# martinruenz/co-fusion

Measured on AMD Instinct MI355X. Metric: frames/sec at 640x480 (N active models) + ICP-reduce achieved HBM GB/s vs peak, higher is better.
Workload: dtype f32

## Files before the change

### co_fusion_amd/api.py

```python
from __future__ import annotations

import ctypes as C

import numpy as np
import torch

from . import lib as _libmod

NUM_PYRS = 3


class Cam(C.Structure):
    _fields_ = [("fx", C.c_float), ("fy", C.c_float), ("cx", C.c_float), ("cy", C.c_float)]

    def level(self, l):
        d = float(1 << l)
        return Cam(self.fx / d, self.fy / d, self.cx / d, self.cy / d)


class Config(C.Structure):
    _fields_ = [("width", C.c_int), ("height", C.c_int), ("fx", C.c_float), ("fy", C.c_float), ("cx", C.c_float),
                ("cy", C.c_float), ("device", C.c_int), ("max_models", C.c_int), ("max_surfels", C.c_int)]


# ... 231 lines not shown
                                         _f(np.asarray(kinv).reshape(9)), _f(np.asarray(krlr).reshape(9)), cols, rows,
                                         A, b, res, sums))
        return (np.array(A, np.float32).reshape(3, 3), np.array(b, np.float32), np.array(res, np.float32),
                np.array(sums, np.int64))

    def gn_solve_step(self, systems, next_level, last_of_level, icp_fix=32):
        arr = systems if isinstance(systems, C.Array) else (GnSystem * len(systems))(*systems)
        self._check(self.lib.cf_gn_solve_step(self.h, len(arr), arr, int(next_level), int(bool(last_of_level)), int(icp_fix)))
        return arr

    def set_icp_launch(self, threads, ppt):
        self._check(self.lib.cf_set_icp_launch(self.h, threads, ppt))

    def set_gn_mode(self, mode):
        self._check(self.lib.cf_set_gn_mode(self.h, int(mode)))

    def track_batch(self, odoms, poses, rgb_only=False, icp_weight=10.0, pyramid=True, fast_odom=False, so3=True, err_surfaces=None):
        n = len(odoms)
        keep = [_f(np.asarray(p, np.float32).reshape(16)) for p in poses]
        pp = (C.POINTER(C.c_float) * max(n, 1))(*[C.cast(k, C.POINTER(C.c_float)) for k in keep])
        oo = (C.c_void_p * max(n, 1))(*[o.h for o in odoms])
        ee = None
        if err_surfaces is not None:
            ee = (C.c_void_p * max(n, 1))(*[e.data_ptr() if e is not None else None for e in err_surfaces])
        opts = TrackOpts(int(rgb_only), int(pyramid), int(fast_odom), int(so3), icp_weight)
        self._check(self.lib.cf_odom_track_batch_async(self.h, oo, n, pp, C.byref(opts), ee))

    def _batch_args(self, odoms, poses):
        n = len(odoms)
        self._keep_poses = [_f(np.asarray(p, np.float32).reshape(16)) for p in poses]
# ... 376 lines not shown
```

### co_fusion_amd/csrc/cabi.hip

```cpp
#include <stdlib.h>
#include <string.h>

#include <string>

#include "cf_host.h"

using namespace cf;

void cf_ctx::set_error(const std::string& m)
{
    std::lock_guard<std::mutex> lk(error_mutex);
    last_error = m;
}

static int lane_ready(cf_ctx* ctx, int lane)
{
    if (!ctx->lanes[lane]) {
        HIPCHK(ctx, hipStreamCreateWithFlags(&ctx->lanes[lane], hipStreamNonBlocking));
        HIPCHK(ctx, hipEventCreateWithFlags(&ctx->lane_done[lane], hipEventDisableTiming));
    }
    return CF_OK;
}
static void leave_lane(cf_ctx* ctx)
{
// ... 23 lines not shown
    ctx->icp_launch = IcpLaunch{256, 0, 0};
    if (int r = dmalloc(ctx, &ctx->d_acc_a, (size_t)kGroups * 32)) return r;
    if (int r = dmalloc(ctx, &ctx->d_acc_b, (size_t)kGroups * 32)) return r;
    if (int r = dmalloc(ctx, &ctx->d_out, 64)) return r;
    if (int r = dmalloc(ctx, &ctx->d_scratch_state, 1)) return r;
    if (int r = dmalloc(ctx, &ctx->d_state_pool, (size_t)cf_ctx::kStateSlots)) return r;
    HIPCHK(ctx, hipHostMalloc(reinterpret_cast<void**>(&ctx->h_state_pool), sizeof(OdomDev) * cf_ctx::kStateSlots, hipHostMallocCoherent));
    memset(ctx->h_state_pool, 0, sizeof(OdomDev) * cf_ctx::kStateSlots);
    if (int r = dmalloc(ctx, &ctx->d_so3_sync, (size_t)ctx->cfg.max_models + 1)) return r;
    if (const char* e = getenv("CF_ICP_ARITH")) {
        if (cf_set_icp_arith(ctx, (!strcmp(e, "gram") || !strcmp(e, "1")) ? CF_ICP_ARITH_GRAM : (!strcmp(e, "reference") || !strcmp(e, "2")) ? CF_ICP_ARITH_REFERENCE
                                  : (!strcmp(e, "product") || !strcmp(e, "0")) ? CF_ICP_ARITH_PRODUCT : -1) != CF_OK) {
            ctx->set_error("CF_ICP_ARITH: product | gram | reference"); return CF_EINVAL;
        }
    }
    if (int r = dmalloc(ctx, &ctx->d_cand_scratch, (size_t)cfg->width * cfg->height)) return r;
    HIPCHK(ctx, hipHostMalloc(reinterpret_cast<void**>(&ctx->h_scratch_state), sizeof(OdomDev)));
    HIPCHK(ctx, hipHostMalloc(reinterpret_cast<void**>(&ctx->h_out), sizeof(unsigned long long) * 64));
    ctx->prof.capacity = 8192;
    ctx->prof.events = new hipEvent_t[ctx->prof.capacity];
    for (int i = 0; i < ctx->prof.capacity; i++) HIPCHK(ctx, hipEventCreate(&ctx->prof.events[i]));
    ctx->prof.used = 0; ctx->prof.enabled = 0; ctx->prof.bytes = 0; ctx->prof.launches = 0;
    HIPCHK(ctx, hipStreamSynchronize(ctx->stream));
    return CF_OK;
}

void cf_destroy(cf_ctx* ctx)
{
    if (ctx && ctx->batch_event) (void)hipEventDestroy(ctx->batch_event);
    if (ctx) for (int i = 0; i < cf_ctx::kSurfEvents; i++) if (ctx->surf_events[i]) (void)hipEventDestroy(ctx->surf_events[i]);
// ... 237 lines not shown
```

### co_fusion_amd/csrc/cabi_track.hip

```cpp
#include <math.h>
#include <stdio.h>
#include <stdlib.h>
#include <string.h>

#include <string>
#include <utility>

#include "cf_host.h"

using namespace cf;

#ifdef CF_ABLATE
static bool diag_no_box() { static const bool v = getenv("CF_NO_SCREEN_BOX") != nullptr; return v; }
static bool diag_no_zcull() { static const bool v = getenv("CF_NO_ZCULL") != nullptr; return v; }
static bool diag_no_occ() { static const bool v = getenv("CF_NO_OCC") != nullptr; return v; }
static const char* diag_icp_ablate() { return getenv("CF_ICP_ABLATE"); }
static const char* diag_trace_out(const char* name) { const char* e = getenv("CF_ICP_TRACE_OUT"); return e ? e : name; }
struct DiagCall {
    const char* name; int call = -2, seen = 0;
    bool hit() { if (call == -2) call = getenv(name) ? atoi(getenv(name)) : -1; return call >= 0 && seen++ == call; }
};
static int clear_accumulators(cf_ctx* ctx, cf_odom* const* ods, int n)
{
    for (int m = 0; m < n; m++) {
// ... 235 lines not shown
    GnHook hook{};
    hook.fn = ctx->collective; hook.user = ctx->collective_user;
    bool any_split = false;
    for (int m = 0; m < n; m++) { hook.split[m] = ods[m]->band_end > 0 ? 1 : 0; any_split = any_split || hook.split[m]; }
    if (any_split && !ctx->collective) { ctx->set_error("a tracker has a row band (cf_odom_set_band) but no collective is registered (cf_set_collective)"); return CF_ESTATE; }
    if (any_split && ctx->gn_mode == 0) { ctx->set_error("split reductions need the record-slot data path (cf_set_gn_mode 1)"); return CF_ESTATE; }
    cf::ProfSink* prof = nullptr;
    if (ctx->prof.enabled > 0 && (ctx->prof_calls++ % (unsigned)ctx->prof.enabled) == 0) prof = &ctx->prof;
    TrackDiag diag;
    if (int r = diag.begin(ctx)) return r;
    LaunchShape* shapes[kMaxBatch];
    for (int m = 0; m < n; m++) shapes[m] = &ods[m]->launch_shape;
    IcpLaunch launch_cfg = ctx->icp_launch; launch_cfg.shape = shapes;
    if (!launch_gn_track(ctx->stream, launch_cfg, states, ctx->d_so3_sync, any_split ? &hook : nullptr, icp_args, rgb_args, n,
                         ctx->cfg.width, ctx->cfg.height, opts->so3 != 0, opts->pyramid != 0, opts->fast_odom != 0, terms.rgb, terms.icp, ctx->gn_mode, prof,
                         h_states, prep_fused ? &prep : nullptr)) {
        ctx->set_error("tracking: the registered collective failed inside the Gauss-Newton loop");
        return CF_ESTATE;
    }
    LAUNCHCHK(ctx);
    if (int r = diag.end(ctx, ods, n, icp_args[0], rgb_args[0])) return r;
    for (int m = 0; m < n; m++) ods[m]->result_pending = true;
    return CF_OK;
}

int cf_wait_stream(cf_ctx* ctx)
{
    HIPCHK(ctx, hipStreamSynchronize(ctx->stream));
    return CF_OK;
}

// ... 43 lines not shown
            for (int r = k + 1; r < N; r++) lu[r * N + k] /= lu[k * N + k];
        for (int r = k + 1; r < N; r++)
            for (int c = k + 1; c < N; c++) lu[r * N + c] -= lu[r * N + k] * lu[k * N + c];
    }
    for (int j = 0; j < N; j++) {
        double x[N];
        for (int i = 0; i < N; i++) x[i] = (perm[i] == j) ? 1.0 : 0.0;
        for (int i = 0; i < N; i++)
            for (int c = 0; c < i; c++) x[i] -= lu[i * N + c] * x[c];
        for (int i = N - 1; i >= 0; i--) {
            for (int c = i + 1; c < N; c++) x[i] -= lu[i * N + c] * x[c];
            x[i] /= lu[i * N + i];
        }
        for (int i = 0; i < N; i++) cov[i * N + j] = x[i];
    }
    return CF_OK;
}

int cf_set_gn_mode(cf_ctx* ctx, int mode)
{
    if (!ctx || mode < 0 || mode > 2) return CF_EINVAL;
    if (mode == 2) {
        if (ctx->xcd_round_robin < 0) { HIPCHK(ctx, hipStreamSynchronize(ctx->stream)); ctx->xcd_round_robin = probe_xcd_round_robin(ctx->stream) ? 1 : 0; }
        if (!ctx->xcd_round_robin) { ctx->set_error("cf_set_gn_mode 2: workgroups of a launch are not dealt round-robin over 8 XCDs on this device; the mode needs that"); return CF_ESTATE; }
    }
    if (mode != ctx->gn_mode) {
        ctx->gn_mode_epoch++;
    }
    ctx->gn_mode = mode;
    return CF_OK;
// ... 38 lines not shown
```

### co_fusion_amd/csrc/cf_host.h

```cpp
#pragma once

#include <string.h>

#include <mutex>
#include <string>

#include "cf_kernels.h"

struct cf_ctx;
struct cf_thread_binding { const cf_ctx* ctx = nullptr; hipStream_t stream = nullptr; };
extern thread_local cf_thread_binding cf_tls_binding;

struct cf_ctx {
    cf_config cfg{};
    hipStream_t stream = nullptr;
    hipStream_t cur() const { return cf_tls_binding.ctx == this ? cf_tls_binding.stream : stream; }
    hipStream_t own_stream = nullptr;
    std::string last_error;
    std::mutex error_mutex;
    cf::IcpLaunch icp_launch{256, 0};
    int icp_arith = 0;
    float* d_ref = nullptr;
    float* h_ref = nullptr;
    unsigned long long* d_acc_a = nullptr;
    unsigned long long* d_acc_b = nullptr;
    unsigned long long* d_out = nullptr;
    unsigned long long* h_out = nullptr;
    cf::OdomDev* d_scratch_state = nullptr;
    cf::OdomDev* h_scratch_state = nullptr;
    uint8_t* d_cand_scratch = nullptr;
    cf::So3Sync* d_so3_sync = nullptr;
    unsigned gn_mode_epoch = 0;
    int xcd_round_robin = -1;
    int gn_mode = 1;
    static constexpr int kStateSlots = 256;
    cf::OdomDev* d_state_pool = nullptr;
    cf::OdomDev* h_state_pool = nullptr;
    bool slot_used[kStateSlots]{};
    hipEvent_t batch_event = nullptr;
    bool extent_cull = true;
    static constexpr int kLanes = 8;
    hipStream_t lanes[kLanes]{};
    hipEvent_t lane_done[kLanes]{};
    hipEvent_t fork_point = nullptr;
    static constexpr int kMarks = 64;
    hipEvent_t marks[kMarks]{};
    bool mark_set[kMarks]{};
    hipStream_t forked_from = nullptr;
    bool forked = false;
    unsigned lanes_used = 0;
    int (*collective)(void* user, int op, void* dev_buf, uint64_t words, void* stream) = nullptr;
    void* collective_user = nullptr;
    void* rccl = nullptr;
    unsigned prof_calls = 0;
// ... 106 lines not shown
```

### co_fusion_amd/csrc/cf_kernels.h

```cpp
#pragma once

#include <hip/hip_runtime.h>
#include <hip/hip_ext.h>
#include <stdint.h>

#include "../../include/cofusion_hip.h"

namespace cf {

__host__ __device__ __forceinline__ cf_cam cam_level(cf_cam c, int level)
{
    const int div = 1 << level;
    return cf_cam{c.fx / div, c.fy / div, c.cx / div, c.cy / div};
}

constexpr int kGroups = 64;

struct alignas(64) GnHot {
    int icp, level_done; float cull_z[2];
    float Rcurr[9], tcurr[3];
    float Rprev_inv[9], tprev[3];
    int cull_box[4];
    int rgb, rgbOnly, level_done2, pad;
    float krkInv[9], kt[3];
// ... 215 lines not shown
void launch_rgb_residual(hipStream_t s, const RgbArgs& ra, int n);
void launch_rgb_step(hipStream_t s, const RgbArgs& ra, int n);
constexpr uint64_t kRgbResidualBytes = 27;
constexpr uint64_t kRgbResidualBytesCompact = 11;
void launch_acc_total(hipStream_t s, const unsigned long long* acc, unsigned long long* out);
void launch_rgb_cand(hipStream_t s, const int16_t* dIdx, const int16_t* dIdy, const float* next_depth,
                     const uint8_t* next_image, float min_scale, int cols, int rows, uint8_t* cand);
void launch_so3_step(hipStream_t s, const uint8_t* last_image, const uint8_t* next_image, const float basis[9],
                     const float kinv[9], const float krlr[9], int cols, int rows, unsigned long long* out16);
void launch_gn_solve(hipStream_t s, const GnArgs& gn, int n, int next_level, int last_of_level);

struct ProfSink {
    hipEvent_t* events; int capacity; int used; uint64_t bytes; uint64_t launches; int enabled;
};

constexpr int kSo3Blocks = 16;
constexpr int kStepSubs = 16;
struct So3Sync { unsigned long long acc[10][16]; unsigned arrive, depart;
                 unsigned step_top, pad;
                 unsigned step_sub[kStepSubs][32]; };
struct GnHook { int (*fn)(void* user, int op, void* dev_buf, uint64_t words, void* stream); void* user; int split[kMaxBatch]; };
struct TrackerStates { OdomDev* dev[kMaxBatch]; const OdomDev* host[kMaxBatch]; };
bool launch_gn_track(hipStream_t s, IcpLaunch cfg, const TrackerStates& states, So3Sync* so3_syncs ,
                     const GnHook* hook, const IcpArgs icp_args[3], const RgbArgs rgb_args[3], int n, int width, int height, bool so3,
                     bool pyramid, bool fast_odom, bool rgb, bool icp, int mode, ProfSink* prof,
                     OdomDev* const* h_states = nullptr ,
                     const RgbPrepBatch* prep = nullptr );
void rgb_prep_levels(RgbPrepBatch& b, int n, int W, int H);
float replay_icp_level0(hipStream_t s, IcpLaunch cfg, const IcpArgs& a0, const RgbArgs& r0, int n, int slots, int ablate, int reps, hipEvent_t e0, hipEvent_t e1);
#ifdef CF_ABLATE
void trace_so3_dump(hipStream_t s);
void trace_solve_begin();
void trace_solve_end(hipStream_t s, const char* path);
void trace_step_solve(hipStream_t s, IcpLaunch cfg, const IcpArgs& a0, const RgbArgs& r0, So3Sync* syncs, int n, const char* path);
void trace_icp_level0(hipStream_t s, IcpLaunch cfg, const IcpArgs& a0, const RgbArgs& r0, int n, int slots, const char* path);
#endif
bool probe_xcd_round_robin(hipStream_t s);
float sqrt_gate_lt(float T);
float sqrt_gate_le(float T);

constexpr int kSurfBatch = 16;
struct IndexPassArgs {
// ... 116 lines not shown
```

### co_fusion_amd/csrc/track_reduce.hip

```cpp
#include "cf_device.h"
#include "cf_kernels.h"
#include "track_prep_dev.h"
#include "track_sums_dev.h"

namespace cf {

__device__ __forceinline__ int idiv(int n, IDiv d) { return (int)(__umulhi((unsigned)n, d.M) >> d.s); }

struct IcpProj { f3 vcurr_g; int g; int inb; int ux, uy; };

__device__ __forceinline__ IcpProj icp_project(const m33& Rcurr, const f3& tcurr, const m33& Rprev_inv, const f3& tprev, const cf_cam& intr,
                                               int cols, int rows, f3 vcurr)
{
    IcpProj o;
    o.vcurr_g = mul(Rcurr, vcurr) + tcurr;
    const f3 vcurr_cp = mul(Rprev_inv, o.vcurr_g - tprev);
    const int ux = f2i_rn(vcurr_cp.x * intr.fx / vcurr_cp.z + intr.cx);
    const int uy = f2i_rn(vcurr_cp.y * intr.fy / vcurr_cp.z + intr.cy);
    o.inb = !(ux < 0 || uy < 0 || ux >= cols || uy >= rows || vcurr_cp.z < 0);
    o.g = o.inb ? uy * cols + ux : 0;
    o.ux = o.inb ? ux : 0; o.uy = o.inb ? uy : 0;
    return o;
}

// ... 660 lines not shown
    g_last_icp_args = args; g_last_n_icp_blocks = n_icp_blocks; g_last_grid = (int)grid.x;
#endif
    const unsigned lds = cfg.gram ? (unsigned)(cfg.threads / 64) * kGramWaveDwords * sizeof(int) : 0u;
    const int tag = (level == 0 ? 0 : level == 1 ? 1 : 2) + (n > 1 ? 4 : 0), ppt_index = cfg.ppt == 4 ? 2 : cfg.ppt == 2 ? 1 : 0;
    static_assert(kIcpKernels[3][0][0] == nullptr && kIcpKernels[2][2][1] && kIcpKernels[4][0][0], "tags are level (0..2) or level + 4: row 3 is never looked up");
    launch_plain_or_timed(kIcpKernels[tag][ppt_index][cfg.gram ? 1 : 0], grid, dim3(cfg.threads), lds, s, ev0, ev1, args, ra, n_icp_blocks);
}

void launch_icp_level(hipStream_t s, IcpLaunch cfg, const IcpArgs& args, int n, int level, hipEvent_t ev0, hipEvent_t ev1)
{
    launch_icp_rgbres(s, cfg, args, RgbArgs{}, true, false, n, level, ev0, ev1);
}

bool launch_gn_track(hipStream_t s, IcpLaunch cfg, const TrackerStates& states, So3Sync* so3_syncs, const GnHook* hook, const IcpArgs icp_args[3],
                     const RgbArgs rgb_args[3], int n, int width, int height, bool so3, bool pyramid, bool fast_odom, bool rgb, bool icp, int mode,
                     ProfSink* prof, OdomDev* const* h_states, const RgbPrepBatch* prep)
{
    int iterations[3];
    iterations[0] = fast_odom ? 3 : 10;
    iterations[1] = pyramid ? 5 : 0;
    iterations[2] = pyramid ? 4 : 0;
    int first_level = 2;
    while (first_level > 0 && iterations[first_level] == 0) first_level--;
    {
        const int gx = so3 ? 8 * kSo3Blocks : 1;
        static const RgbPrepBatch none{};
        const int prep_bx = prep ? prep->m[0].L.blk_end[2] : 0;
        so3_prealign_kernel<<<gx * n + prep_bx * n, 256, 0, s>>>(states, so3_syncs, so3 ? 1 : 0, first_level, gx, gx * n, prep ? *prep : none, prep_bx);
    }
    GnArgs gn{};
    gn.icp_gram = cfg.gram;
    gn.slot_px = cfg.threads * 4;
    for (int m = 0; m < n; m++) {
        gn.od[m] = const_cast<OdomDev*>(icp_args[0].m[m].st);
        gn.icp_acc[m] = icp_args[0].m[m].acc;
        gn.rgb_acc[m] = rgb_args[0].m[m].rgb_acc;
        gn.od_host[m] = h_states ? h_states[m] : nullptr;
    }
    const bool slots = mode != 0;
    bool any_culled = false;
    for (int m = 0; m < n; m++) any_culled = any_culled || (icp_args[0].m[m].cull && icp_args[0].m[m].err);
    const bool err_aside = icp && any_culled;
    bool hook_failed = false;
// ... 211 lines not shown
```

### co_fusion_amd/csrc/track_so3_dev.h

```cpp
#pragma once
#include "track_prep_dev.h"
#include "track_sums_dev.h"

namespace cf {

__device__ __forceinline__ void screen_box(const float* lo, const float* hi, const float* Rb, const float* tb, const float* Rcurr, const float* tcurr,
                                           cf_cam intr, float distThres, int W, int H, int lane, int (&out)[4], float (&zout)[2])
{
    const float finf = __int_as_float(0x7f800000);
    zout[0] = -finf; zout[1] = finf;
    if (!(lo[0] <= hi[0])) { out[0] = 1; out[1] = 1; out[2] = 0; out[3] = 0; return; }
    const float m = distThres * 1.01f + 1e-3f;
    const float px = (lane & 1) ? hi[0] + 3.f : lo[0] - 3.f, py = (lane & 2) ? hi[1] + 3.f : lo[1] - 3.f;
    const float znear = lo[2] - m, pz = (lane & 4) ? hi[2] + m : znear;
    const float cx_ = (px - intr.cx) / intr.fx * pz, cy_ = (py - intr.cy) / intr.fy * pz;
    const float dx = (Rb[0] * cx_ + Rb[1] * cy_ + Rb[2] * pz + tb[0]) - tcurr[0];
    const float dy = (Rb[3] * cx_ + Rb[4] * cy_ + Rb[5] * pz + tb[1]) - tcurr[1];
    const float dz = (Rb[6] * cx_ + Rb[7] * cy_ + Rb[8] * pz + tb[2]) - tcurr[2];
    const float xc = Rcurr[0] * dx + Rcurr[3] * dy + Rcurr[6] * dz;
    const float yc = Rcurr[1] * dx + Rcurr[4] * dy + Rcurr[7] * dz;
    const float zc = Rcurr[2] * dx + Rcurr[5] * dy + Rcurr[8] * dz;
    const float u = intr.fx * xc / zc + intr.cx, v = intr.fy * yc / zc + intr.cy;
    const bool bad = !(znear > 0.05f) || !(zc > 0.05f) || !is_finite(u) || !is_finite(v);
    float u0 = u, u1 = u, v0 = v, v1 = v, z0 = zc, z1 = zc;
// ... 7 lines not shown
    zout[0] = z0 - (1e-3f + 1e-3f * fabsf(z0)); zout[1] = z1 + (1e-3f + 1e-3f * fabsf(z1));
    const float fw = (float)(W + 16), fh = (float)(H + 16);
    out[0] = (int)floorf(fminf(fmaxf(u0, -16.f), fw)) - 3; out[1] = (int)floorf(fminf(fmaxf(v0, -16.f), fh)) - 3;
    out[2] = (int)ceilf(fminf(fmaxf(u1, -16.f), fw)) + 3; out[3] = (int)ceilf(fminf(fmaxf(v1, -16.f), fh)) + 3;
}

__device__ __forceinline__ void so3_gradient(const uint8_t* __restrict__ img, int cols, int x, int y, float& gx, float& gy)
{
    const float actu = (float)img[y * cols + x];
    float back = (float)img[y * cols + x - 1], fore = (float)img[y * cols + x + 1];
    gx = ((back + actu) / 2.0f) - ((fore + actu) / 2.0f);
    back = (float)img[(y - 1) * cols + x]; fore = (float)img[(y + 1) * cols + x];
    gy = ((back + actu) / 2.0f) - ((fore + actu) / 2.0f);
}

__device__ __forceinline__ void so3_pass(const uint8_t* __restrict__ lastImage, const uint8_t* __restrict__ nextImage,
                                         const m33& B, const m33& Ki, const float* __restrict__ krlr, int cols, int rows,
                                         unsigned long long (*lds)[16], unsigned long long* totals, int block, int blocks)
{
    constexpr float lim = (float)(1 << ((50 - kFixSO3) / 2));
    constexpr float scale = (float)(1 << kFixSO3);
    const int N = cols * rows, T = blockDim.x;
    unsigned long long acc[16];
#pragma unroll
    for (int k = 0; k < 16; k++) acc[k] = 0;
    const float a = krlr[0], b = krlr[1], c = krlr[2], d = krlr[3], e = krlr[4], f = krlr[5], g = krlr[6], h = krlr[7],
                ii = krlr[8];
    for (int k = block * T + threadIdx.x; k < N; k += blocks * T) {
        const int y = k / cols, x = k - y * cols;
        const f3 unwarped = {(float)x, (float)y, 1.0f};
        const f3 warped = mul(B, unwarped);
        const int wx = f2i_rn(warped.x / warped.z), wy = f2i_rn(warped.y / warped.z);
        if (!(wx >= 1 && wx < cols - 1 && wy >= 1 && wy < rows - 1 && x >= 1 && x < cols - 1 && y >= 1 && y < rows - 1))
            continue;
        float gnx, gny, glx, gly;
        so3_gradient(nextImage, cols, wx, wy, gnx, gny);
        so3_gradient(lastImage, cols, x, y, glx, gly);
        const float gx = (gnx + glx) / 2.0f, gy = (gny + gly) / 2.0f;
        const f3 point = mul(Ki, unwarped);
        const float z2 = point.z * point.z;
        const f3 left = {((point.z * (d * gy + a * gx)) - (gy * g * y) - (gx * g * x)) / z2,
                         ((point.z * (e * gy + b * gx)) - (gy * h * y) - (gx * h * x)) / z2,
                         ((point.z * (f * gy + c * gx)) - (gy * ii * y) - (gx * ii * x)) / z2};
        const f3 jac = cross(left, point);
        const float row[4] = {jac.x, jac.y, jac.z, -((float)nextImage[wy * cols + wx] - (float)lastImage[y * cols + x])};
        double r[4], rs[4];
#pragma unroll
        for (int q = 0; q < 4; q++) { r[q] = (double)clamp_row(row[q], lim); rs[q] = (double)(clamp_row(row[q], lim) * scale); }
#pragma unroll
        for (int p = 0; p < 3; p++)
#pragma unroll
            for (int q = 0; q < 4; q++)
                if (q >= p)
                    acc[4 * p - (p * (p - 1)) / 2 + (q - p)] += (unsigned long long)__double_as_longlong(fma(rs[p], r[q], kMagic)) - kMagicBits;
        acc[9] += (unsigned long long)__double_as_longlong(fma(rs[3], r[3], kMagic)) - kMagicBits;
        acc[10] += 1;
    }
    const int lane = threadIdx.x & 63, wave = threadIdx.x >> 6;
    const unsigned long long v = wave_reduce16_u64(acc, lane);
    if ((lane & 3) == 0) lds[wave][lane >> 2] = v;
    __syncthreads();
    if (threadIdx.x < 16) {
        unsigned long long t = 0;
        for (int w = 0; w < (T >> 6); w++) t += lds[w][threadIdx.x];
        totals[threadIdx.x] = t;
    }
    __syncthreads();
}

__device__ inline void so3_unpack(const unsigned long long* t, float A[9], float b[3], float residual[2])
{
    int shift = 0;
    for (int i = 0; i < 3; ++i)
        for (int j = i; j < 4; ++j) {
            const float value = fix_to_f32((long long)t[shift++], kFixSO3);
            if (j == 3) b[i] = value;
            else A[j * 3 + i] = A[i * 3 + j] = value;
        }
    residual[0] = fix_to_f32((long long)t[9], kFixSO3);
    residual[1] = (float)(long long)t[10];
}

// ... 22 lines not shown
                                                        const uint8_t* __restrict__ nextImage, m33 B, m33 Ki, m33 krlr,
                                                        int cols, int rows, unsigned long long* __restrict__ out16)
{
    __shared__ unsigned long long lds[16][16];
    __shared__ unsigned long long totals[16];
    so3_pass(lastImage, nextImage, B, Ki, krlr.m, cols, rows, lds, totals, blockIdx.x, gridDim.x);
    if (threadIdx.x < 16) out16[threadIdx.x] = totals[threadIdx.x];
}

#ifdef CF_ABLATE
__device__ unsigned long long g_so3_trace[12][8];
#define OSTAMP(it, k) do { if (lead && by == 0 && threadIdx.x == 0) g_so3_trace[it][k] = wall_clock64(); } while (0)
#else
#define OSTAMP(it, k) do {} while (0)
#endif
__global__ void __launch_bounds__(256) so3_prealign_kernel(const TrackerStates ts, So3Sync* __restrict__ syncs, int do_so3,
                                                           int first_level, int gx, int so3_blocks, const RgbPrepBatch prep, int prep_bx)
{
    if ((int)blockIdx.x >= so3_blocks) {
        const int r = (int)blockIdx.x - so3_blocks, m = r / prep_bx;
        rgb_prep_body(prep.m[m], r - m * prep_bx);
        return;
    }
    const int by = (int)blockIdx.x / gx, bxx = (int)blockIdx.x - by * gx;
    OdomDev* const god = ts.dev[by];
    So3Sync* sync = syncs + by;
    __shared__ OdomDev s_od;
    __shared__ unsigned long long lds[16][16];
    __shared__ unsigned long long totals[16];
    __shared__ float s_basis[9], s_kinv[9], s_krlr[9];
    __shared__ int s_done;
    __shared__ double s_resultR[9];
    __shared__ double s_K[9], s_Kinv[9];
    __shared__ float s_Rlr[9];
    __shared__ float s_lastError, s_lastCount;
    __shared__ double s_lastResultR[9];
    __shared__ float s_jtj[9], s_jtr[3], s_delta[3], s_fws[15];
    __shared__ int s_iws[3];
    const bool one_xcd = do_so3 && gx > 1;
    if (one_xcd && (bxx & 7) != (by & 7)) return;
    const int bx = one_xcd ? (bxx >> 3) : bxx;
    const bool lead = bx == 0;
    const unsigned G = one_xcd ? (unsigned)gx >> 3 : (unsigned)gx;
    {
        static_assert(sizeof(OdomDev) % 4 == 0, "OdomDev is staged as 32-bit words");
        constexpr int kWords = (int)(sizeof(OdomDev) / 4);
        const unsigned* __restrict__ src = reinterpret_cast<const unsigned*>(ts.host[by]);
        constexpr int kPer = (kWords + 255) / 256;
        unsigned w[kPer];
#pragma unroll
        for (int q = 0; q < kPer; q++) w[q] = ((int)threadIdx.x + 256 * q < kWords) ? src[threadIdx.x + 256 * q] : 0u;
#pragma unroll
        for (int q = 0; q < kPer; q++) if ((int)threadIdx.x + 256 * q < kWords) reinterpret_cast<unsigned*>(&s_od)[threadIdx.x + 256 * q] = w[q];
        __syncthreads();
        if (lead) for (int k = threadIdx.x; k < kWords; k += 256) reinterpret_cast<unsigned*>(god)[k] = reinterpret_cast<const unsigned*>(&s_od)[k];
        __syncthreads();
    }
    const OdomDev* const od = &s_od;
    const int L = 2, cols = od->width >> L, rows = od->height >> L;
    if (threadIdx.x == 0) {
        for (int k = 0; k < 9; k++) { s_resultR[k] = (k % 4 == 0) ? 1.0 : 0.0; s_lastResultR[k] = s_resultR[k]; s_Rlr[k] = (k % 4 == 0) ? 1.f : 0.f; }
        k_matrix(cam_level(od->intr, L), s_K);
        inv33<double>(s_K, s_Kinv);
        s_lastError = 3.402823466e+38F / 2; s_lastCount = 3.402823466e+38F / 2;
        s_done = 0;
        if (lead) { god->stats.so3_iterations = 0; god->stats.last_so3_error = 0; god->stats.last_so3_count = 0; }
    }
    __syncthreads();
    if (do_so3) {
        const uint8_t* __restrict__ lastNext = od->lastNextImage[L];
        const uint8_t* __restrict__ next = od->nextImage[L];
        OSTAMP(11, 0);
        for (int it = 0; it < 10; it++) {
            OSTAMP(it, 0);
            if (threadIdx.x == 0) {
                double tmp[9], H[9];
                mul33<double>(s_K, s_resultR, tmp);
                mul33<double>(tmp, s_Kinv, H);
                for (int k = 0; k < 9; k++) { s_basis[k] = (float)H[k]; s_kinv[k] = (float)s_Kinv[k]; s_krlr[k] = (float)tmp[k]; }
            }
            __syncthreads();
            m33 B, Ki;
            for (int k = 0; k < 9; k++) { B.m[k] = s_basis[k]; Ki.m[k] = s_kinv[k]; }
            OSTAMP(it, 1);
            so3_pass(lastNext, next, B, Ki, s_krlr, cols, rows, lds, totals, bx, (int)G);
            OSTAMP(it, 2);
            if (G > 1) {
                if (threadIdx.x < 64) {
                    unsigned long long* slot = sync->acc[it];
                    if (threadIdx.x < 11 && totals[threadIdx.x] != 0)
                        __hip_atomic_fetch_add(&slot[threadIdx.x], totals[threadIdx.x], __ATOMIC_RELAXED, __HIP_MEMORY_SCOPE_WORKGROUP);
                    asm volatile("s_waitcnt vmcnt(0)" ::: "memory");
                    if (threadIdx.x == 0) {
                        __hip_atomic_fetch_add(&sync->arrive, 1u, __ATOMIC_RELAXED, __HIP_MEMORY_SCOPE_WORKGROUP);
                        const unsigned target = (unsigned)(it + 1) * G;
                        unsigned spins = 0;
                        while (l2_read_u32(&sync->arrive) < target) {
                            if (++spins > (1u << 22)) { god->stats.fault = 1; break; }
                            __builtin_amdgcn_s_sleep(1);
                        }
// ... 82 lines not shown
```

### co_fusion_amd/lib.py

```python
from __future__ import annotations

import ctypes as C
import os
import subprocess

_HERE = os.path.dirname(os.path.abspath(__file__))
_LIB_DIR = os.environ.get("CF_LIB_DIR") or os.path.join(_HERE, "lib")
LIB_PATH = os.environ.get("CF_HIP_LIB") or os.path.join(_LIB_DIR, "libcofusion_hip.so")

SYMBOLS = [
    "cf_create", "cf_destroy", "cf_last_error", "cf_set_stream", "cf_use_own_stream", "cf_get_stream", "cf_synchronize", "cf_fork", "cf_main", "cf_join", "cf_join_lane", "cf_thread_lane", "cf_mark", "cf_event_wait_host", "cf_fork_after", "cf_malloc",
    "cf_free", "cf_memcpy_h2d", "cf_memcpy_d2h", "cf_malloc_host", "cf_free_host", "cf_memcpy_h2d_async", "cf_memcpy_d2h_async", "cf_memcpy_d2d_async", "cf_rgb_to_rgba", "cf_create_vmap", "cf_create_nmap", "cf_copy_maps", "cf_resize_map",
    "cf_transform_maps", "cf_vertices_to_depth", "cf_pyrdown_gauss_f32", "cf_pyrdown_gauss_u8",
    "cf_rgba_to_intensity", "cf_sobel", "cf_project_cloud", "cf_icp_step", "cf_icp_step_band", "cf_rgb_residual", "cf_rgb_step",
    "cf_so3_step", "cf_gn_solve_step", "cf_odom_create", "cf_odom_destroy", "cf_odom_init_icp_model", "cf_odom_init_rgb_model",
    "cf_odom_init_rgb", "cf_odom_init_models_batch", "cf_odom_init_models_batch_frames", "cf_odom_init_models_batch_select", "cf_model_fill_ratio_device", "cf_odom_init_first_rgb", "cf_odom_init_icp", "cf_odom_init_icp_maps", "cf_odom_get_incremental_transformation",
    "cf_odom_track_batch_async", "cf_odom_fetch_result", "cf_odom_get_covariance", "cf_odom_bind_frame_maps", "cf_odom_share_frame_maps", "cf_odom_set_culling", "cf_odom_set_band", "cf_set_collective", "cf_model_predict_indices_sharded", "cf_odom_buffer",
    "cf_bilateral", "cf_model_create", "cf_model_destroy", "cf_model_initialise", "cf_model_count",
    "cf_model_predict_indices", "cf_model_index_keys", "cf_model_index_resolve", "cf_model_combined_predict", "cf_model_predict_inactive", "cf_model_synthesize_depth", "cf_model_prefetch_fill_ratio", "cf_model_perform_fill_in", "cf_model_requires_fill_in",
    "cf_model_fuse", "cf_model_clean", "cf_models_frame_passes", "cf_models_preindex", "cf_model_download_map", "cf_model_upload_map", "cf_model_buffer",
    "cf_set_extent_culling", "cf_model_extents_unknown",
    "cf_redetect_score", "cf_redetect_timing", "cf_relabel",
    "cf_fusion_weight", "cf_seg_create", "cf_seg_destroy", "cf_seg_slic", "cf_seg_crf", "cf_seg_sums", "cf_seg_infer", "cf_seg_early", "cf_seg_run_batch", "cf_seg_fetch", "cf_seg_publish_poses", "cf_seg_fetch_poses",
    "cf_seg_labels", "cf_seg_buffer", "cf_seg_create_masks", "cf_seg_masks", "cf_seg_masks_batch", "cf_seg_new_mask_value",
    "cf_depth_pyramid", "cf_set_icp_launch", "cf_set_icp_arith", "cf_get_icp_arith", "cf_set_gn_mode", "cf_profile_enable", "cf_profile_read", "cf_odom_bench_icp", "cf_odom_level0_visited", "cf_odom_last_launch_shape",
    "cf_rccl_unique_id", "cf_rccl_init", "cf_rccl_allreduce", "cf_rccl_broadcast", "cf_rccl_info", "cf_rccl_destroy",
    "cf_render_create", "cf_render_destroy", "cf_render", "cf_render_palette",
    "cf_ferns_table", "cf_ferns_create", "cf_ferns_destroy", "cf_ferns_get_table", "cf_ferns_encode", "cf_ferns_search", "cf_ferns_append", "cf_ferns_add_async",
    "cf_ferns_relocalise", "cf_ferns_count", "cf_ferns_download", "cf_ferns_last_search",
    "cf_frame_decoder_create", "cf_frame_decoder_destroy", "cf_frame_decoder_slot", "cf_frame_decoder_submit", "cf_frame_decoder_acquire", "cf_frame_decoder_timing",
    "cf_frame_decoder_enable_images", "cf_frame_decoder_image_slot", "cf_frame_decoder_submit_images", "cf_frame_decoder_acquire_mask", "cf_frame_decoder_image_timing",
    "cf_png_encoder_create", "cf_png_encoder_destroy", "cf_png_encoder_submit", "cf_png_encoder_acquire", "cf_png_encoder_timing",
    "cf_deform_create", "cf_deform_destroy", "cf_deform_default_thresholds", "cf_deform_sample", "cf_deform_set_nodes", "cf_deform_weights", "cf_deform_assemble",
    "cf_deform_iterate", "cf_deform_optimise", "cf_deform_apply", "cf_deform_apply_poses", "cf_deform_download", "cf_deform_weights_device",
    "cf_deform_create_sized", "cf_deform_assemble_local", "cf_deform_iterate_local", "cf_deform_optimise_local",
    "cf_ferns_gate_async", "cf_ferns_gate_wait", "cf_ferns_constraints", "cf_ferns_find_frame", "cf_ferns_constraint_buffers", "cf_ferns_keyframe_buffers",
    "cf_local_loop_create", "cf_local_loop_destroy", "cf_local_loop_constraints_async", "cf_local_loop_wait", "cf_local_loop_constraint_buffers",
]


# ... 70 lines not shown
```

### include/cofusion_hip.h

```cpp
#ifndef COFUSION_HIP_H_
#define COFUSION_HIP_H_

#include <stdint.h>

#ifdef __cplusplus
extern "C" {
#endif

#define CF_OK 0
#define CF_EINVAL (-1)
#define CF_EHIP (-2)
#define CF_ENOMEM (-3)
#define CF_ESTATE (-4)

#define CF_NUM_PYRS 3
#define CF_SE3_WORDS 32
#define CF_SO3_WORDS 16
#define CF_FIX_ICP 32
#define CF_FIX_RGB_MAX 32
static inline int CF_FIX_RGB_BITS(float sigma)
{
    union { float f; uint32_t u; } v;
    int F;
    if (sigma == -1.0f || !(sigma >= 2.0f)) return 8;
// ... 297 lines not shown
    const uint8_t *mask_dev;
    const float *depth_dev;
    int32_t n_models;
    const uint32_t *model_ids;
    uint32_t next_model_id;
    int32_t allow_new;
    const uint8_t *mapping;
    uint8_t *full_dev;
} cf_seg_mask_job;
int cf_seg_create_masks(cf_ctx *ctx, cf_segmenter **out);
int cf_seg_masks(const cf_seg_mask_job *job);
int cf_seg_masks_batch(cf_ctx *ctx, const cf_seg_mask_job *jobs, int n_jobs);
int cf_seg_new_mask_value(cf_segmenter *s, int *value);

int cf_set_gn_mode(cf_ctx *ctx, int mode);
int cf_set_icp_launch(cf_ctx *ctx, int threads, int pixels_per_thread);
#define CF_ICP_ARITH_PRODUCT 0
#define CF_ICP_ARITH_GRAM 1
#define CF_ICP_ARITH_REFERENCE 2
int cf_set_icp_arith(cf_ctx *ctx, int mode);
int cf_get_icp_arith(cf_ctx *ctx);

typedef struct cf_renderer cf_renderer;
#define CF_RENDER_MAX_ITEMS 256
#define CF_RENDER_MAX_COLOUR 8
#define CF_RENDER_UNSTABLE 1
#define CF_RENDER_WINDOW 2
#define CF_RENDER_PHONG 4
#define CF_RENDER_GREY 0
#define CF_RENDER_NORMALS 1
// ... 215 lines not shown
```

Measured before the change: 942.2.

## Stage SO3 prealign next-image in LDS and keep last-image gradients in registers

The SO3 prealignment kernel now copies the level-2 next image (up to 160x120) into shared memory once and precomputes per-thread packed last-image intensity and gradients into registers. Each of the ten Gauss-Newton iterations then reads from LDS and registers instead of re-reading both images from global memory. Uniform matrix values are broadcast with readfirstlane, and the launch bounds ask for more waves per SIMD. The 19 KB of static LDS can lower occupancy. Gradients are quantised to half-pixel steps in 9 bits, which could change results slightly if gradients exceed that range.

```diff
diff --git a/co_fusion_amd/api.py b/co_fusion_amd/api.py
--- a/co_fusion_amd/api.py
+++ b/co_fusion_amd/api.py
@@ -269,6 +269,9 @@
 
     def set_gn_mode(self, mode):
         self._check(self.lib.cf_set_gn_mode(self.h, int(mode)))
+
+    def set_so3_onchip(self, on=True):
+        self._check(self.lib.cf_set_so3_onchip(self.h, int(bool(on))))
 
     def track_batch(self, odoms, poses, rgb_only=False, icp_weight=10.0, pyramid=True, fast_odom=False, so3=True, err_surfaces=None):
         n = len(odoms)
diff --git a/co_fusion_amd/csrc/cabi.hip b/co_fusion_amd/csrc/cabi.hip
--- a/co_fusion_amd/csrc/cabi.hip
+++ b/co_fusion_amd/csrc/cabi.hip
@@ -61,6 +61,7 @@
             ctx->set_error("CF_ICP_ARITH: product | gram | reference"); return CF_EINVAL;
         }
     }
+    ctx->so3_onchip = getenv("CF_NO_SO3_ONCHIP") == nullptr;
     if (int r = dmalloc(ctx, &ctx->d_cand_scratch, (size_t)cfg->width * cfg->height)) return r;
     HIPCHK(ctx, hipHostMalloc(reinterpret_cast<void**>(&ctx->h_scratch_state), sizeof(OdomDev)));
     HIPCHK(ctx, hipHostMalloc(reinterpret_cast<void**>(&ctx->h_out), sizeof(unsigned long long) * 64));
diff --git a/co_fusion_amd/csrc/cabi_track.hip b/co_fusion_amd/csrc/cabi_track.hip
--- a/co_fusion_amd/csrc/cabi_track.hip
+++ b/co_fusion_amd/csrc/cabi_track.hip
@@ -273,7 +273,7 @@
     IcpLaunch launch_cfg = ctx->icp_launch; launch_cfg.shape = shapes;
     if (!launch_gn_track(ctx->stream, launch_cfg, states, ctx->d_so3_sync, any_split ? &hook : nullptr, icp_args, rgb_args, n,
                          ctx->cfg.width, ctx->cfg.height, opts->so3 != 0, opts->pyramid != 0, opts->fast_odom != 0, terms.rgb, terms.icp, ctx->gn_mode, prof,
-                         h_states, prep_fused ? &prep : nullptr)) {
+                         h_states, prep_fused ? &prep : nullptr, ctx->so3_onchip)) {
         ctx->set_error("tracking: the registered collective failed inside the Gauss-Newton loop");
         return CF_ESTATE;
     }
@@ -347,6 +347,13 @@
         }
         for (int i = 0; i < N; i++) cov[i * N + j] = x[i];
     }
+    return CF_OK;
+}
+
+int cf_set_so3_onchip(cf_ctx* ctx, int on)
+{
+    if (!ctx) return CF_EINVAL;
+    ctx->so3_onchip = on != 0;
     return CF_OK;
 }
 
diff --git a/co_fusion_amd/csrc/cf_host.h b/co_fusion_amd/csrc/cf_host.h
--- a/co_fusion_amd/csrc/cf_host.h
+++ b/co_fusion_amd/csrc/cf_host.h
@@ -38,6 +38,7 @@
     cf::OdomDev* h_state_pool = nullptr;
     bool slot_used[kStateSlots]{};
     hipEvent_t batch_event = nullptr;
+    bool so3_onchip = true;
     bool extent_cull = true;
     static constexpr int kLanes = 8;
     hipStream_t lanes[kLanes]{};
diff --git a/co_fusion_amd/csrc/cf_kernels.h b/co_fusion_amd/csrc/cf_kernels.h
--- a/co_fusion_amd/csrc/cf_kernels.h
+++ b/co_fusion_amd/csrc/cf_kernels.h
@@ -253,7 +253,16 @@
     hipEvent_t* events; int capacity; int used; uint64_t bytes; uint64_t launches; int enabled;
 };
 
-constexpr int kSo3Blocks = 16;
+#ifndef CF_SO3_BLOCKS
+#define CF_SO3_BLOCKS 16
+#endif
+constexpr int kSo3Blocks = CF_SO3_BLOCKS;
+constexpr int kSo3LdsImage = 160 * 120;
+#ifndef CF_SO3_WAVES
+#define CF_SO3_WAVES 5
+#endif
+constexpr int kSo3Waves = CF_SO3_WAVES;
+constexpr int kSo3Keep = (kSo3LdsImage + kSo3Blocks * 256 - 1) / (kSo3Blocks * 256);
 constexpr int kStepSubs = 16;
 struct So3Sync { unsigned long long acc[10][16]; unsigned arrive, depart;
                  unsigned step_top, pad;
@@ -264,7 +273,8 @@
                      const GnHook* hook, const IcpArgs icp_args[3], const RgbArgs rgb_args[3], int n, int width, int height, bool so3,
                      bool pyramid, bool fast_odom, bool rgb, bool icp, int mode, ProfSink* prof,
                      OdomDev* const* h_states = nullptr ,
-                     const RgbPrepBatch* prep = nullptr );
+                     const RgbPrepBatch* prep = nullptr ,
+                     bool so3_onchip = true );
 void rgb_prep_levels(RgbPrepBatch& b, int n, int W, int H);
 float replay_icp_level0(hipStream_t s, IcpLaunch cfg, const IcpArgs& a0, const RgbArgs& r0, int n, int slots, int ablate, int reps, hipEvent_t e0, hipEvent_t e1);
 #ifdef CF_ABLATE
diff --git a/co_fusion_amd/csrc/track_reduce.hip b/co_fusion_amd/csrc/track_reduce.hip
--- a/co_fusion_amd/csrc/track_reduce.hip
+++ b/co_fusion_amd/csrc/track_reduce.hip
@@ -698,7 +698,7 @@
 
 bool launch_gn_track(hipStream_t s, IcpLaunch cfg, const TrackerStates& states, So3Sync* so3_syncs, const GnHook* hook, const IcpArgs icp_args[3],
                      const RgbArgs rgb_args[3], int n, int width, int height, bool so3, bool pyramid, bool fast_odom, bool rgb, bool icp, int mode,
-                     ProfSink* prof, OdomDev* const* h_states, const RgbPrepBatch* prep)
+                     ProfSink* prof, OdomDev* const* h_states, const RgbPrepBatch* prep, bool so3_onchip)
 {
     int iterations[3];
     iterations[0] = fast_odom ? 3 : 10;
@@ -710,7 +710,7 @@
         const int gx = so3 ? 8 * kSo3Blocks : 1;
         static const RgbPrepBatch none{};
         const int prep_bx = prep ? prep->m[0].L.blk_end[2] : 0;
-        so3_prealign_kernel<<<gx * n + prep_bx * n, 256, 0, s>>>(states, so3_syncs, so3 ? 1 : 0, first_level, gx, gx * n, prep ? *prep : none, prep_bx);
+        so3_prealign_kernel<<<gx * n + prep_bx * n, 256, 0, s>>>(states, so3_syncs, so3 ? (so3_onchip ? 3 : 1) : 0, first_level, gx, gx * n, prep ? *prep : none, prep_bx);
     }
     GnArgs gn{};
     gn.icp_gram = cfg.gram;
diff --git a/co_fusion_amd/csrc/track_so3_dev.h b/co_fusion_amd/csrc/track_so3_dev.h
--- a/co_fusion_amd/csrc/track_so3_dev.h
+++ b/co_fusion_amd/csrc/track_so3_dev.h
@@ -45,18 +45,57 @@
     gy = ((back + actu) / 2.0f) - ((fore + actu) / 2.0f);
 }
 
+__device__ __forceinline__ void so3_pixel(unsigned long long (&acc)[16], float gnx, float gny, float glx, float gly, float nextValue, float lastValue,
+                                          int x, int y, const m33& Ki, const float* __restrict__ krlr)
+{
+    constexpr float lim = (float)(1 << ((50 - kFixSO3) / 2));
+    constexpr float scale = (float)(1 << kFixSO3);
+    const float a = krlr[0], b = krlr[1], c = krlr[2], d = krlr[3], e = krlr[4], f = krlr[5], g = krlr[6], h = krlr[7],
+                ii = krlr[8];
+    const f3 unwarped = {(float)x, (float)y, 1.0f};
+    const float gx = (gnx + glx) / 2.0f, gy = (gny + gly) / 2.0f;
+    const f3 point = mul(Ki, unwarped);
+    const float z2 = point.z * point.z;
+    const f3 left = {((point.z * (d * gy + a * gx)) - (gy * g * y) - (gx * g * x)) / z2,
+                     ((point.z * (e * gy + b * gx)) - (gy * h * y) - (gx * h * x)) / z2,
+                     ((point.z * (f * gy + c * gx)) - (gy * ii * y) - (gx * ii * x)) / z2};
+    const f3 jac = cross(left, point);
+    const float row[4] = {jac.x, jac.y, jac.z, -(nextValue - lastValue)};
+    double r[4], rs[4];
+#pragma unroll
+    for (int q = 0; q < 4; q++) { r[q] = (double)clamp_row(row[q], lim); rs[q] = (double)(clamp_row(row[q], lim) * scale); }
+#pragma unroll
+    for (int p = 0; p < 3; p++)
+#pragma unroll
+        for (int q = 0; q < 4; q++)
+            if (q >= p)
+                acc[4 * p - (p * (p - 1)) / 2 + (q - p)] += (unsigned long long)__double_as_longlong(fma(rs[p], r[q], kMagic)) - kMagicBits;
+    acc[9] += (unsigned long long)__double_as_longlong(fma(rs[3], r[3], kMagic)) - kMagicBits;
+    acc[10] += 1;
+}
+
+__device__ __forceinline__ void so3_pass_totals(const unsigned long long (&acc)[16], unsigned long long (*lds)[16], unsigned long long* totals)
+{
+    const int lane = threadIdx.x & 63, wave = threadIdx.x >> 6, T = blockDim.x;
+    const unsigned long long v = wave_reduce16_u64(acc, lane);
+    if ((lane & 3) == 0) lds[wave][lane >> 2] = v;
+    __syncthreads();
+    if (threadIdx.x < 16) {
+        unsigned long long t = 0;
+        for (int w = 0; w < (T >> 6); w++) t += lds[w][threadIdx.x];
+        totals[threadIdx.x] = t;
+    }
+    __syncthreads();
+}
+
 __device__ __forceinline__ void so3_pass(const uint8_t* __restrict__ lastImage, const uint8_t* __restrict__ nextImage,
                                          const m33& B, const m33& Ki, const float* __restrict__ krlr, int cols, int rows,
                                          unsigned long long (*lds)[16], unsigned long long* totals, int block, int blocks)
 {
-    constexpr float lim = (float)(1 << ((50 - kFixSO3) / 2));
-    constexpr float scale = (float)(1 << kFixSO3);
     const int N = cols * rows, T = blockDim.x;
     unsigned long long acc[16];
 #pragma unroll
     for (int k = 0; k < 16; k++) acc[k] = 0;
-    const float a = krlr[0], b = krlr[1], c = krlr[2], d = krlr[3], e = krlr[4], f = krlr[5], g = krlr[6], h = krlr[7],
-                ii = krlr[8];
     for (int k = block * T + threadIdx.x; k < N; k += blocks * T) {
         const int y = k / cols, x = k - y * cols;
         const f3 unwarped = {(float)x, (float)y, 1.0f};
@@ -67,36 +106,69 @@
         float gnx, gny, glx, gly;
         so3_gradient(nextImage, cols, wx, wy, gnx, gny);
         so3_gradient(lastImage, cols, x, y, glx, gly);
-        const float gx = (gnx + glx) / 2.0f, gy = (gny + gly) / 2.0f;
-        const f3 point = mul(Ki, unwarped);
-        const float z2 = point.z * point.z;
-        const f3 left = {((point.z * (d * gy + a * gx)) - (gy * g * y) - (gx * g * x)) / z2,
-                         ((point.z * (e * gy + b * gx)) - (gy * h * y) - (gx * h * x)) / z2,
-                         ((point.z * (f * gy + c * gx)) - (gy * ii * y) - (gx * ii * x)) / z2};
-        const f3 jac = cross(left, point);
-        const float row[4] = {jac.x, jac.y, jac.z, -((float)nextImage[wy * cols + wx] - (float)lastImage[y * cols + x])};
-        double r[4], rs[4];
-#pragma unroll
-        for (int q = 0; q < 4; q++) { r[q] = (double)clamp_row(row[q], lim); rs[q] = (double)(clamp_row(row[q], lim) * scale); }
-#pragma unroll
-        for (int p = 0; p < 3; p++)
-#pragma unroll
-            for (int q = 0; q < 4; q++)
-                if (q >= p)
-                    acc[4 * p - (p * (p - 1)) / 2 + (q - p)] += (unsigned long long)__double_as_longlong(fma(rs[p], r[q], kMagic)) - kMagicBits;
-        acc[9] += (unsigned long long)__double_as_longlong(fma(rs[3], r[3], kMagic)) - kMagicBits;
-        acc[10] += 1;
-    }
-    const int lane = threadIdx.x & 63, wave = threadIdx.x >> 6;
-    const unsigned long long v = wave_reduce16_u64(acc, lane);
-    if ((lane & 3) == 0) lds[wave][lane >> 2] = v;
-    __syncthreads();
-    if (threadIdx.x < 16) {
-        unsigned long long t = 0;
-        for (int w = 0; w < (T >> 6); w++) t += lds[w][threadIdx.x];
-        totals[threadIdx.x] = t;
-    }
-    __syncthreads();
+        so3_pixel(acc, gnx, gny, glx, gly, (float)nextImage[wy * cols + wx], (float)lastImage[y * cols + x], x, y, Ki, krlr);
+    }
+    so3_pass_totals(acc, lds, totals);
+}
+
+struct So3Kept { unsigned px[kSo3Keep], xy[kSo3Keep]; };
+__device__ __forceinline__ float so3_uniform(float v) { return __int_as_float(__builtin_amdgcn_readfirstlane(__float_as_int(v))); }
+constexpr unsigned kSo3Interior = 1u << 26;
+
+__device__ __forceinline__ void so3_keep(So3Kept& kept, const uint8_t* __restrict__ lastImage, int cols, int rows, int block, int blocks)
+{
+    const int N = cols * rows;
+#pragma unroll
+    for (int j = 0; j < kSo3Keep; j++) {
+        const int k = (block + j * blocks) * 256 + (int)threadIdx.x;
+        const int y = k / cols, x = k - y * cols;
+        kept.px[j] = 0; kept.xy[j] = (unsigned)x | ((unsigned)y << 16);
+        if (k < N && x >= 1 && x < cols - 1 && y >= 1 && y < rows - 1) {
+            float glx, gly;
+            so3_gradient(lastImage, cols, x, y, glx, gly);
+            kept.px[j] = kSo3Interior | ((unsigned)lastImage[y * cols + x] << 18) | (((unsigned)(int)(gly * 2.0f) & 0x1ffu) << 9) | ((unsigned)(int)(glx * 2.0f) & 0x1ffu);
+        }
+    }
+}
+
+__device__ __forceinline__ void so3_stage_next(uint8_t* s_next, const uint8_t* __restrict__ nextImage, int N)
+{
+    constexpr int kPer = (kSo3LdsImage / 16 + 255) / 256;
+    const uint4* __restrict__ src = reinterpret_cast<const uint4*>(nextImage);
+    const int chunks = N >> 4;
+    uint4 w[kPer];
+#pragma unroll
+    for (int q = 0; q < kPer; q++) w[q] = ((int)threadIdx.x + 256 * q < chunks) ? src[threadIdx.x + 256 * q] : make_uint4(0, 0, 0, 0);
+    const int t = (chunks << 4) + (int)threadIdx.x;
+    if (t < N) s_next[t] = nextImage[t];
+#pragma unroll
+    for (int q = 0; q < kPer; q++) if ((int)threadIdx.x + 256 * q < chunks) reinterpret_cast<uint4*>(s_next)[threadIdx.x + 256 * q] = w[q];
+}
+
+__device__ __forceinline__ void so3_pass_onchip(const So3Kept& kept, const uint8_t* s_next, const m33& B, const m33& Ki, const float* __restrict__ krlr,
+                                                int cols, int rows, unsigned long long (*lds)[16], unsigned long long* totals)
+{
+    unsigned long long acc[16];
+#pragma unroll
+    for (int k = 0; k < 16; k++) acc[k] = 0;
+#pragma unroll 1
+    for (int j = 0; j < kSo3Keep; j++) {
+        unsigned p = kept.px[0], xy = kept.xy[0];
+#pragma unroll
+        for (int q = 1; q < kSo3Keep; q++) if (j == q) { p = kept.px[q]; xy = kept.xy[q]; }
+        if (!(p & kSo3Interior)) continue;
+        const int x = (int)(xy & 0xffffu), y = (int)(xy >> 16);
+        const f3 unwarped = {(float)x, (float)y, 1.0f};
+        const f3 warped = mul(B, unwarped);
+        const int wx = f2i_rn(warped.x / warped.z), wy = f2i_rn(warped.y / warped.z);
+        if (!(wx >= 1 && wx < cols - 1 && wy >= 1 && wy < rows - 1))
+            continue;
+        float gnx, gny;
+        so3_gradient(s_next, cols, wx, wy, gnx, gny);
+        const float glx = (float)((int)(p << 23) >> 23) / 2.0f, gly = (float)((int)(p << 14) >> 23) / 2.0f;
+        so3_pixel(acc, gnx, gny, glx, gly, (float)s_next[wy * cols + wx], (float)((p >> 18) & 0xffu), x, y, Ki, krlr);
+    }
+    so3_pass_totals(acc, lds, totals);
 }
 
 __device__ inline void so3_unpack(const unsigned long long* t, float A[9], float b[3], float residual[2])
@@ -149,7 +221,7 @@
 #else
 #define OSTAMP(it, k) do {} while (0)
 #endif
-__global__ void __launch_bounds__(256) so3_prealign_kernel(const TrackerStates ts, So3Sync* __restrict__ syncs, int do_so3,
+__global__ void __launch_bounds__(256, kSo3Waves) so3_prealign_kernel(const TrackerStates ts, So3Sync* __restrict__ syncs, int so3_flags,
                                                            int first_level, int gx, int so3_blocks, const RgbPrepBatch prep, int prep_bx)
 {
     if ((int)blockIdx.x >= so3_blocks) {
@@ -157,6 +229,7 @@
         rgb_prep_body(prep.m[m], r - m * prep_bx);
         return;
     }
+    const bool do_so3 = (so3_flags & 1) != 0;
     const int by = (int)blockIdx.x / gx, bxx = (int)blockIdx.x - by * gx;
     OdomDev* const god = ts.dev[by];
     So3Sync* sync = syncs + by;
@@ -177,6 +250,9 @@
     const int bx = one_xcd ? (bxx >> 3) : bxx;
     const bool lead = bx == 0;
     const unsigned G = one_xcd ? (unsigned)gx >> 3 : (unsigned)gx;
+    __shared__ __attribute__((aligned(16))) uint8_t s_next[kSo3LdsImage];
+    So3Kept kept;
+    bool onchip;
     {
         static_assert(sizeof(OdomDev) % 4 == 0, "OdomDev is staged as 32-bit words");
         constexpr int kWords = (int)(sizeof(OdomDev) / 4);
@@ -189,14 +265,24 @@
         for (int q = 0; q < kPer; q++) if ((int)threadIdx.x + 256 * q < kWords) reinterpret_cast<unsigned*>(&s_od)[threadIdx.x + 256 * q] = w[q];
         __syncthreads();
         if (lead) for (int k = threadIdx.x; k < kWords; k += 256) reinterpret_cast<unsigned*>(god)[k] = reinterpret_cast<const unsigned*>(&s_od)[k];
-        __syncthreads();
     }
     const OdomDev* const od = &s_od;
     const int L = 2, cols = od->width >> L, rows = od->height >> L;
+    {
+        const unsigned N = (unsigned)(cols * rows);
+        onchip = do_so3 && (so3_flags & 2) && N <= (unsigned)kSo3LdsImage && (N + G * 256 - 1) / (G * 256) <= (unsigned)kSo3Keep &&
+                 (reinterpret_cast<uintptr_t>(od->nextImage[L]) & 15) == 0;
+        if (onchip) {
+            so3_stage_next(s_next, od->nextImage[L], (int)N);
+            so3_keep(kept, od->lastNextImage[L], cols, rows, bx, (int)G);
+        }
+        __syncthreads();
+    }
     if (threadIdx.x == 0) {
         for (int k = 0; k < 9; k++) { s_resultR[k] = (k % 4 == 0) ? 1.0 : 0.0; s_lastResultR[k] = s_resultR[k]; s_Rlr[k] = (k % 4 == 0) ? 1.f : 0.f; }
         k_matrix(cam_level(od->intr, L), s_K);
         inv33<double>(s_K, s_Kinv);
+        for (int k = 0; k < 9; k++) s_kinv[k] = (float)s_Kinv[k];
         s_lastError = 3.402823466e+38F / 2; s_lastCount = 3.402823466e+38F / 2;
         s_done = 0;
         if (lead) { god->stats.so3_iterations = 0; god->stats.last_so3_error = 0; god->stats.last_so3_count = 0; }
@@ -205,6 +291,8 @@
     if (do_so3) {
         const uint8_t* __restrict__ lastNext = od->lastNextImage[L];
         const uint8_t* __restrict__ next = od->nextImage[L];
+        m33 Ki;
+        for (int k = 0; k < 9; k++) Ki.m[k] = onchip ? so3_uniform(s_kinv[k]) : s_kinv[k];
         OSTAMP(11, 0);
         for (int it = 0; it < 10; it++) {
             OSTAMP(it, 0);
@@ -212,13 +300,18 @@
                 double tmp[9], H[9];
                 mul33<double>(s_K, s_resultR, tmp);
                 mul33<double>(tmp, s_Kinv, H);
-                for (int k = 0; k < 9; k++) { s_basis[k] = (float)H[k]; s_kinv[k] = (float)s_Kinv[k]; s_krlr[k] = (float)tmp[k]; }
+                for (int k = 0; k < 9; k++) { s_basis[k] = (float)H[k]; s_krlr[k] = (float)tmp[k]; }
             }
             __syncthreads();
-            m33 B, Ki;
-            for (int k = 0; k < 9; k++) { B.m[k] = s_basis[k]; Ki.m[k] = s_kinv[k]; }
+            m33 B;
+            for (int k = 0; k < 9; k++) B.m[k] = s_basis[k];
             OSTAMP(it, 1);
-            so3_pass(lastNext, next, B, Ki, s_krlr, cols, rows, lds, totals, bx, (int)G);
+            if (onchip) {
+                m33 Bu, Krlr;
+                for (int k = 0; k < 9; k++) { Bu.m[k] = so3_uniform(B.m[k]); Krlr.m[k] = so3_uniform(s_krlr[k]); }
+                so3_pass_onchip(kept, s_next, Bu, Ki, Krlr.m, cols, rows, lds, totals);
+            }
+            else so3_pass(lastNext, next, B, Ki, s_krlr, cols, rows, lds, totals, bx, (int)G);
             OSTAMP(it, 2);
             if (G > 1) {
                 if (threadIdx.x < 64) {
diff --git a/co_fusion_amd/lib.py b/co_fusion_amd/lib.py
--- a/co_fusion_amd/lib.py
+++ b/co_fusion_amd/lib.py
@@ -23,7 +23,7 @@
     "cf_redetect_score", "cf_redetect_timing", "cf_relabel",
     "cf_fusion_weight", "cf_seg_create", "cf_seg_destroy", "cf_seg_slic", "cf_seg_crf", "cf_seg_sums", "cf_seg_infer", "cf_seg_early", "cf_seg_run_batch", "cf_seg_fetch", "cf_seg_publish_poses", "cf_seg_fetch_poses",
     "cf_seg_labels", "cf_seg_buffer", "cf_seg_create_masks", "cf_seg_masks", "cf_seg_masks_batch", "cf_seg_new_mask_value",
-    "cf_depth_pyramid", "cf_set_icp_launch", "cf_set_icp_arith", "cf_get_icp_arith", "cf_set_gn_mode", "cf_profile_enable", "cf_profile_read", "cf_odom_bench_icp", "cf_odom_level0_visited", "cf_odom_last_launch_shape",
+    "cf_depth_pyramid", "cf_set_icp_launch", "cf_set_icp_arith", "cf_get_icp_arith", "cf_set_gn_mode", "cf_set_so3_onchip", "cf_profile_enable", "cf_profile_read", "cf_odom_bench_icp", "cf_odom_level0_visited", "cf_odom_last_launch_shape",
     "cf_rccl_unique_id", "cf_rccl_init", "cf_rccl_allreduce", "cf_rccl_broadcast", "cf_rccl_info", "cf_rccl_destroy",
     "cf_render_create", "cf_render_destroy", "cf_render", "cf_render_palette",
     "cf_ferns_table", "cf_ferns_create", "cf_ferns_destroy", "cf_ferns_get_table", "cf_ferns_encode", "cf_ferns_search", "cf_ferns_append", "cf_ferns_add_async",
diff --git a/include/cofusion_hip.h b/include/cofusion_hip.h
--- a/include/cofusion_hip.h
+++ b/include/cofusion_hip.h
@@ -335,6 +335,7 @@
 int cf_seg_new_mask_value(cf_segmenter *s, int *value);
 
 int cf_set_gn_mode(cf_ctx *ctx, int mode);
+int cf_set_so3_onchip(cf_ctx *ctx, int on);
 int cf_set_icp_launch(cf_ctx *ctx, int threads, int pixels_per_thread);
 #define CF_ICP_ARITH_PRODUCT 0
 #define CF_ICP_ARITH_GRAM 1
```

Result: no change. 950.7, median of 6 (+0.9%).
